# Lexmata/llama-gguf

Hardware: AMD Instinct MI355X
Metric: decode tokens/sec Llama-3-8B Q4_K_M, 1 GPU; % of HBM roofline (higher is better)
Workload: dtype f32 (x as 4xint8 limbs on the matrix cores, exact int32 accumulation)

## Files before the change

### include/llama_gguf_hip.h

```cpp
#ifndef LLAMA_GGUF_HIP_H
#define LLAMA_GGUF_HIP_H

#include <stddef.h>
#include <stdint.h>

#ifdef __cplusplus
extern "C" {
#endif

typedef enum lgh_status {
  LGH_OK = 0,
  LGH_NOT_AVAILABLE = 1,
  LGH_SHAPE_MISMATCH = 2,
  LGH_DTYPE_MISMATCH = 3,
  LGH_UNSUPPORTED_DTYPE = 4,
  LGH_UNSUPPORTED = 5,
  LGH_INVALID_ARGUMENT = 6,
  LGH_TENSOR_ERROR = 7,
  LGH_INITIALIZATION_FAILED = 8,
  LGH_ALLOCATION_FAILED = 9,
  LGH_OPERATION_FAILED = 10
} lgh_status;

typedef enum lgh_ggml_type {
// ... 29 lines not shown
enum {
  LGH_KV_F32 = 0,
  LGH_KV_INT8 = 1,
  LGH_KV_FP8_E4M3 = 2,
  LGH_KV_FP8_E5M2 = 3,
  LGH_KV_TQ2 = 4,
  LGH_KV_TQ3 = 5,
  LGH_KV_TQ2_QJL = 6,
  LGH_KV_TQ3_QJL = 7,
};

enum {
  LGH_FLAG_NO_GRAPH = 1u << 0,
  LGH_FLAG_EXACT_PREFILL = 1u << 2,
  LGH_FLAG_KV_INT8 = 1u << 4,
  LGH_FLAG_REMOVED_MASK = (1u << 1) | (1u << 3) | (1u << 5) | (1u << 6) | (1u << 7) | (0xFFu << 24),
  LGH_FLAG_ATTN_SPLITS_SHIFT = 8,
  LGH_FLAG_ATTN_DIRECT_SHIFT = 16
};

typedef struct lgh_ctx lgh_ctx;

enum {
  LGH_K_EMBED = 0, LGH_K_QKV = 1, LGH_K_ATTN = 2, LGH_K_ATTN_COMBINE = 3, LGH_K_WO = 4, LGH_K_GATEUP = 5,
  LGH_K_DOWN = 6, LGH_K_ROUTER = 7, LGH_K_OUTPUT = 8, LGH_K_ARGMAX = 9, LGH_K_MISC = 10,
  LGH_K_TOKEN = 11,
  LGH_K_COUNT = 16
};

enum {
  LGH_SYM_MV_Q4K = 0,
// ... 5 lines not shown
  LGH_SYM_MV_Q5K_Q6K = 6,
  LGH_SYM_MV_ALL = 7,
  LGH_SYM_F32_MATVEC = 8,
  LGH_SYM_ATTN = 9,
  LGH_SYM_ATTN_COMBINE = 10,
  LGH_SYM_EMBED = 11,
  LGH_SYM_ARGMAX = 12,
  LGH_SYM_ROUTER = 13,
  LGH_SYM_OTHER = 14,
  LGH_SYM_MVQ_Q4K = 15,
  LGH_SYM_MVQ_Q6K = 16,
  LGH_SYM_MVQ_MIXED = 17,
  LGH_SYM_MVQ_Q5K = 18,
  LGH_SYM_MVQ_Q80_Q40 = 19,
  LGH_SYM_PTOK = 20,
  LGH_SYM_COUNT = 24
};

typedef struct lgh_stats {
  uint64_t weight_bytes;
  uint64_t kv_bytes;
  uint64_t scratch_bytes;
  uint64_t tokens_processed;
  uint64_t graph_nodes;
  uint64_t k_launches[LGH_K_COUNT];
  double k_time_us[LGH_K_COUNT];
  uint64_t k_alg_bytes[LGH_K_COUNT];
  uint64_t sym_launches[LGH_SYM_COUNT];
  double sym_time_us[LGH_SYM_COUNT];
  uint64_t sym_alg_bytes[LGH_SYM_COUNT];
// ... 122 lines not shown
                            size_t n_kv_heads, size_t head_dim, size_t max_seq_len, float scale, size_t pos, int n_splits);
int lgh_op_attention_kv8(int device, uint32_t kv_cache_type, const float* q, int8_t* k_bytes, int8_t* v_bytes, float* k_scale, float* v_scale,
                         const float* k_new, const float* v_new, float* out, size_t n_heads, size_t n_kv_heads, size_t head_dim,
                         size_t max_seq_len, float scale, size_t pos, int n_splits);
int lgh_op_attention_tq(int device, uint32_t kv_cache_type, const float* q, uint8_t* k_codes, uint8_t* v_codes, uint32_t* k_qjl,
                        const float* k_new, const float* v_new, const float* signs, const float* qjl_matrices, float* out, size_t n_heads,
                        size_t n_kv_heads, size_t head_dim, size_t max_seq_len, float scale, size_t pos, int n_splits);
int lgh_op_attention_prefill(int device, const float* q, const float* k_cache, const float* v_cache, float* out, size_t n_heads,
                             size_t n_kv_heads, size_t head_dim, size_t max_seq_len, float scale, size_t pos0, size_t m_tokens);
int lgh_op_qkv_rope(int device, const uint32_t* types, const void* const* w, const float* const* bias, const float* x, const float* norm_w,
                    float eps, size_t hidden, size_t head_dim, size_t n_heads, size_t n_kv_heads, size_t max_seq_len, size_t pos,
                    float rope_base, float rope_scale, float* q_out, float* k_cache, float* v_cache);
int lgh_op_linear_chain(int device, uint32_t type_a, const void* w_a, const void* w_a_up, const float* bias_a, size_t k, size_t n_a,
                        const float* x, const float* norm_w, float eps, const float* resid, int xq_next, const float* next_nw,
                        uint32_t type_b, const void* w_b, size_t n_b, float* out_a, float* out_b, float* out_b_requant, int* image_used);
int lgh_op_moe_experts(int device, uint32_t type_gate_up, const void* w_gate, const void* w_up, uint32_t type_down, const void* w_down,
                       size_t n_experts, size_t hidden, size_t ffn, size_t top_k, const float* router, const int* sel, const float* sel_w,
                       const float* x, const float* norm_w, float eps, float* out, int* sel_out, float* sel_w_out);
typedef struct lgh_backend lgh_backend;
int lgh_backend_create(int device, lgh_backend** out);
void lgh_backend_destroy(lgh_backend* be);
int lgh_backend_load_weight(lgh_backend* be, const char* name, uint32_t ggml_type, const void* w, size_t k, size_t n);
int lgh_backend_has_weight(const lgh_backend* be, const char* name);
int lgh_backend_vec_mat_q(lgh_backend* be, const char* name, const float* x, float* out, size_t k, size_t n);
const char* lgh_backend_last_error(const lgh_backend* be);
int lgh_op_norm_vec_mat(int device, uint32_t ggml_type, const void* w, const float* x, const float* norm_w, float eps,
                        float* out, size_t k, size_t n);
int lgh_op_swiglu_vec_mat(int device, uint32_t ggml_type, const void* w_gate, const void* w_up, const float* x,
                          const float* norm_w, float eps, float* out, size_t k, size_t n);

// ... 31 lines not shown
```

### llama-gguf_amd/csrc/common.h

```cpp
#pragma once

#include <hip/hip_runtime.h>
#include <stdint.h>
#include <stddef.h>
#include <vector>

#include "../../include/llama_gguf_hip.h"

namespace lgh {

typedef uint32_t u32x4 __attribute__((ext_vector_type(4)));
typedef uint32_t u32x2 __attribute__((ext_vector_type(2)));
typedef float f32x4 __attribute__((ext_vector_type(4)));

constexpr int kWave = 64;
constexpr int kNumCU = 256;

__host__ __device__ inline uint32_t blk_elems(int t) {
  switch (t) {
    case LGH_TYPE_F32: case LGH_TYPE_F16: case LGH_TYPE_BF16: return 1;
    case LGH_TYPE_Q4_0: case LGH_TYPE_Q4_1: case LGH_TYPE_Q5_0: case LGH_TYPE_Q5_1: case LGH_TYPE_Q8_0:
    case LGH_TYPE_Q8_1: return 32;
    case LGH_TYPE_Q2_K: case LGH_TYPE_Q3_K: case LGH_TYPE_Q4_K: case LGH_TYPE_Q5_K: case LGH_TYPE_Q6_K:
    case LGH_TYPE_Q8_K: return 256;
// ... 98 lines not shown
  uint32_t ssq_stride;
  uint32_t out_stride[3];
  uint32_t resid_stride[3];
  uint32_t xq_out_stride[3];
  uint32_t ssq_out_stride[3];
  float* part;
  uint64_t part_floats;
  const int* ind_cnt;
  const int* ind_idx;
  uint32_t ind_div;
  uint32_t ind_stride;
  uint32_t ind_nz;
  uint64_t part_z_floats;
};

struct MvGeom { uint32_t wbpack, geom, geom2, red_floats, lds_red_off, n_wg; };

struct MvPlan {
  uint32_t units, T, G, rows_per_wg, n_wg, threads, red_floats;
};

hipError_t mv_plan(int dev_type, uint32_t k, uint32_t n_rows, int npass, MvPlan* plan, uint32_t launch_rows,
                   uint32_t wave_cap);
uint32_t mv_wave_cap(int dev_type);
hipError_t mv_launch(const MvLaunch& L, uint32_t n_wg, uint32_t threads, hipStream_t st);
int mv_symbol(const MvLaunch& L);
hipError_t mvq_plan(uint32_t k, uint32_t n_rows, int npass, MvPlan* plan, uint32_t launch_rows, uint32_t force_tiles = 0);
hipError_t mvq_launch(const MvLaunch& L, uint32_t n_wg, uint32_t threads, hipStream_t st);
hipError_t repack_q4k_t16_launch(const uint8_t* raw, uint8_t* dst, uint32_t n_rows, uint32_t nblk, hipStream_t st);
hipError_t hbm_read_launch(const uint8_t* buf, size_t bytes, float* sink, int nt, hipStream_t st);
uint32_t mvq_pack(const MvLaunch& L, uint32_t n_wg, uint32_t threads, MvGeom* g, size_t* lds_out);
uint32_t mvq_format_mask(const MvLaunch& L);
uint32_t mvq_tile_bytes(int dev_type);
hipError_t mvqb_launch(const MvLaunch& L, const MvBatch& B, uint32_t n_wg, uint32_t threads, hipStream_t st);
size_t mvqb_lds_bytes(uint32_t n_seq, uint32_t red_floats);
hipError_t xq_quantize_launch(const float* x, const float* nw, uint8_t* xq, float* ssq_part, uint32_t k, hipStream_t st);
hipError_t repack_t16_launch(int dev_type, const uint8_t* raw, uint8_t* dst, uint32_t n_rows, uint32_t nblk, hipStream_t st);
hipError_t repack_q6k_t16_launch(const uint8_t* raw, uint8_t* dst, uint32_t n_rows, uint32_t nblk, hipStream_t st);
hipError_t f32_matvec_launch(const float* w, const float* x, float* out, uint32_t k, uint32_t n, const float* norm_w,
                             float eps, const float* resid, hipStream_t st);

hipError_t repack_launch(int src_type, const uint8_t* raw, uint8_t* dst, const uint64_t plane_off[4], uint64_t n_blocks,
                         hipStream_t st);
// ... 74 lines not shown
```

### llama-gguf_amd/csrc/engine.h

```cpp
#pragma once

#include <string>
#include <vector>

#include "common.h"
#include "sample.h"

namespace lgh {

struct LayerW {
  bool owned = false;
  DevWeight wq, wk, wv, wo, gate, up, down;
  DevWeight gate_exps, up_exps, down_exps;
  float* attn_norm = nullptr;
  float* ffn_norm = nullptr;
  float* router = nullptr;
  float* bq = nullptr; float* bk = nullptr; float* bv = nullptr; float* bo = nullptr;
  float* kcache = nullptr;
  float* vcache = nullptr;
  int8_t *k8 = nullptr, *v8 = nullptr;
  float *kscale = nullptr, *vscale = nullptr;
  uint32_t* kx = nullptr;
  bool moe() const { return router != nullptr; }
};
// ... 59 lines not shown
  float* output_norm = nullptr;
  void *fwd_hidden = nullptr, *fwd_token = nullptr;
  float *hidden = nullptr, *xnorm = nullptr, *q = nullptr, *kv_tmp = nullptr, *attn_out = nullptr, *act = nullptr,
        *act2 = nullptr, *logits = nullptr, *part_ml = nullptr, *part_acc = nullptr, *rope_cs = nullptr, *moe_w = nullptr,
        *amax_v = nullptr;
  int *moe_sel = nullptr, *state = nullptr, *amax_i = nullptr, *tok_log = nullptr;
  uint32_t n_splits = 8;
  size_t pos = 0;
  bool finalized = false;
  bool profiling = false;
  std::string err;
  hipGraphExec_t graph[lgh::MODE_COUNT][2] = {};
  bool attn_direct = false;
  uint32_t direct_attn_max_kv = 0;
  uint64_t graph_nodes = 0;
  lgh_stats stats{};
  std::vector<lgh::ProfRec> prof;
  std::vector<void*> allocs;
  std::vector<lgh::XqBuf> xqs;
  lgh::PfScratch pf;
  lgh::BatchScratch batch;
  float* tq_signs = nullptr;
  std::vector<float> tq_signs_host;
  float* tq_qjl = nullptr;
  std::vector<float> tq_qjl_host;
  float* kv_shift_tmp = nullptr;
  lgh::SampBufs samp;
  lgh_sampler_config samp_cfg{};
  bool samp_set = false;
};
// ... 75 lines not shown
```

### llama-gguf_amd/csrc/engine.hip

```cpp
#include "engine.h"
#include "prefill.h"
#include "xq.h"

#include <algorithm>
#include <cmath>
#include <cstdio>
#include <cstdlib>
#include <cstring>

using namespace lgh;

namespace lgh {
hipError_t kv_store_launch(const float* k, const float* v, float* kcache, float* vcache, uint32_t n_kv, uint32_t d,
                           uint32_t max_seq, const int* pos, hipStream_t st);
}

int fail(lgh_ctx* c, int status, const std::string& msg) {
  if (c) c->err = msg;
  return status;
}

#define HIP_TRY(c, status, expr)                                                                      \
  do {                                                                                                \
    hipError_t e__ = (expr);                                                                          \
// ... 290 lines not shown
      } else if (qo && sp.epi != EPI_ROPE_K && sp.epi != EPI_V_CACHE) {
        qo->fresh = false;
      }
      if (sp.out2 && !S.xq_out2) xq_stale(c, sp.out2);
    }
    S.head_dim = c->d.head_dim;
    S.max_seq = c->d.max_seq_len;
    wg += plan.n_wg;
    if (plan.threads > threads) threads = plan.threads;
    if (plan.red_floats > L.red_floats) L.red_floats = plan.red_floats;
  }
  alg += (uint64_t)k * 4 * (norm_w ? 2 : 1);
  return LGH_OK;
}

static int mvq_symbol(const MvLaunch& L) {
  bool has[8] = {false, false, false, false, false, false, false, false};
  for (int s = 0; s < L.nseg; s++) {
    const int t = L.seg[s].type;
    has[t == kDevQ4K_T16 ? 0 : t == kDevQ6K_T16 ? 1 : t == kDevQ5K_T16 ? 2 : t == kDevQ80_T16 ? 3 : 4] = true;
  }
  return has[2] ? LGH_SYM_MVQ_Q5K : (has[3] || has[4]) ? LGH_SYM_MVQ_Q80_Q40 : (has[0] && has[1]) ? LGH_SYM_MVQ_MIXED
         : has[1] ? LGH_SYM_MVQ_Q6K : LGH_SYM_MVQ_Q4K;
}

static int launch_mv_group(lgh_ctx* c, int cls, const SegSpec* specs, int nseg, const float* norm_w, uint32_t k, bool mfma) {
  MvLaunch L;
  uint32_t wg, threads;
  uint64_t alg;
  int rc = build_mv_group(c, specs, nseg, norm_w, k, mfma, L, wg, threads, alg, 0);
  if (rc) return rc;
  if (mfma) return run_k(c, cls, mvq_symbol(L), alg, [&] { return mvq_launch(L, wg, threads, c->stream); });
  return run_k(c, cls, mv_symbol(L), alg, [&] { return mv_launch(L, wg, threads, c->stream); });
}

int launch_mv(lgh_ctx* c, int cls, const SegSpec* specs, int nseg, const float* norm_w, uint32_t k) {
  SegSpec a[3], b[3];
  int na = 0, nb = 0;
  for (int s = 0; s < nseg; s++) {
    if (mfma_type(specs[s].W[0]->type)) a[na++] = specs[s];
    else b[nb++] = specs[s];
  }
  int rc = LGH_OK;
  if (na > 1) {
    bool q4 = false, q5 = false, other = false;
    for (int s = 0; s < na; s++) {
      const int t = a[s].W[0]->type;
// ... 1251 lines not shown
```

### llama-gguf_amd/csrc/matvec_mfma.hip

```cpp
#include <algorithm>
#include <type_traits>

#include "device_utils.h"
#include "mv_epilogue.h"
#include "xq.h"
#include "mvq_core.h"
#include "timeline.h"

LGH_TL_DEFINE(mvq)

namespace lgh {

#ifdef LGH_STAMPS
__device__ unsigned long long g_stamps[8192 * 8];
hipError_t mvq_read_stamps(unsigned long long* host, size_t n) {
  return hipMemcpyFromSymbol(host, HIP_SYMBOL(g_stamps), n * sizeof(unsigned long long));
}
#define LGH_STAMP(i)                                                                             \
  do {                                                                                           \
    if (threadIdx.x == 0 && blockIdx.x < 8192) g_stamps[blockIdx.x * 8 + (i)] = __builtin_amdgcn_s_memrealtime(); \
  } while (0)
__device__ unsigned long long g_wstamps[2048 * 16 * 8];
hipError_t mvq_read_wave_stamps(unsigned long long* host, size_t n) {
  return hipMemcpyFromSymbol(host, HIP_SYMBOL(g_wstamps), n * sizeof(unsigned long long));
// ... 436 lines not shown
  mv_epilogue(L, S, wg, red, ssq, S_T, epi_pre);
  LGH_STAMP(5);
  LGH_WSTAMP(7);
  LGH_SPAN(1);
}

template <uint32_t MASK>
__global__ void __launch_bounds__(kWaves * 64) mvq_kernel(uint32_t wbpack, uint32_t geom, uint32_t geom2, uint32_t L_red_floats,
                                                          uint32_t lds_red_off, const MvLaunch L) {
  extern __shared__ __attribute__((aligned(16))) uint8_t smem8[];
  LGH_TL_BEGIN(mvq, lgh::TL_MVQ, geom2);
  mvq_body<MASK>(blockIdx.x, wbpack, geom, geom2, L_red_floats, lds_red_off, L, smem8);
  LGH_TL_END();
}

hipError_t mvq_plan(uint32_t k, uint32_t n_rows, int npass, MvPlan* plan, uint32_t launch_rows, uint32_t force_tiles) {
  if (k == 0 || k % 256 || n_rows == 0 || npass < 1 || npass > 4) return hipErrorInvalidValue;
  const uint32_t nblk = k / 256, W = kWaves;
  uint32_t T = 1;
  for (uint32_t t = 1; t <= W && t <= nblk; t++)
    if (nblk % t == 0) T = t;
  if (T < W / 2 && nblk > W) T = W;
  if (T > nblk) T = nblk;
  const uint32_t G = W / T >= 1 ? W / T : 1;
  const uint32_t nbw = (nblk + T - 1) / T;
  if (launch_rows < n_rows) launch_rows = n_rows;
  const uint32_t tiles_launch = (launch_rows + 15) / 16;
  uint32_t R = force_tiles ? force_tiles : (tiles_launch + kNumCU - 1) / kNumCU;
  R = (R + G - 1) / G * G;
  const uint32_t threads = T * G * 64;
  const uint32_t rmax = threads / 16 / G * G;
  if (R > rmax) R = rmax;
  plan->units = nbw;
  plan->T = T;
  plan->G = G;
  plan->rows_per_wg = 16 * R;
  plan->n_wg = ((n_rows + 15) / 16 + R - 1) / R;
  plan->threads = threads;
  plan->red_floats = (uint32_t)npass * T * 16 * R;
  return hipSuccess;
}

static uint32_t mvq_red_offset(uint32_t nwaves, uint32_t nbw) { return nwaves * nbw * kXqRecord; }
size_t mvq_lds_bytes(uint32_t nwaves, uint32_t nbw, uint32_t red_floats) {
  return (size_t)mvq_red_offset(nwaves, nbw) + (size_t)red_floats * 4 + 64;
}

template <uint32_t MASK>
static hipError_t mvq_go(const MvLaunch& L, uint32_t n_wg, uint32_t threads, size_t lds, hipStream_t st, uint32_t wbpack, uint32_t geom,
                         uint32_t geom2, uint32_t red_off) {
  static bool attr_set[64] = {};
  if (hipError_t e = lds_opt_in(reinterpret_cast<const void*>(&mvq_kernel<MASK>), 160 * 1024, attr_set); e != hipSuccess) return e;
  hipLaunchKernelGGL((mvq_kernel<MASK>), dim3(n_wg), dim3(threads), lds, st, wbpack, geom, geom2, L.red_floats, red_off, L);
  return hipGetLastError();
}

uint32_t mvq_pack(const MvLaunch& L, uint32_t n_wg, uint32_t threads, MvGeom* g, size_t* lds_out) {
  const MvSeg& S0 = L.seg[0];
  const size_t lds = mvq_lds_bytes(threads / 64, S0.units, L.red_floats);
  if (lds > 160 * 1024 || threads == 0 || threads > kWaves * 64 || n_wg == 0 || L.nseg < 1 || L.nseg > 3) return 0;
  uint32_t mask = 0;
  for (int i = 0; i < L.nseg; i++) {
    const MvSeg& Si = L.seg[i];
    if (Si.T != S0.T || Si.G != S0.G || Si.units != S0.units || Si.nblk != S0.nblk || Si.rows_per_wg % (16 * S0.G) ||
        (i > 0 && Si.wg_begin >= 0xFFFFu))
      return 0;
    const int f = fmt_of_dev_type(Si.type);
    if (f < 0) return 0;
    mask |= 1u << f;
  }
  const uint32_t Rg = S0.rows_per_wg / 16 / S0.G;
  if (S0.T > 255 || S0.G > 255 || S0.units > 0x3FFF || S0.nblk > 0xFFFF || Rg > 0xFFFF) return 0;
  g->wbpack = (L.nseg > 1 ? L.seg[1].wg_begin : 0xFFFFu) | (L.nseg > 2 ? L.seg[2].wg_begin : 0xFFFFu) << 16;
  g->geom = S0.T | S0.G << 8 | S0.units << 16 | (L.do_norm ? 1u << 31 : 0u);
  g->geom2 = S0.nblk | Rg << 16;
  g->red_floats = L.red_floats;
  g->lds_red_off = mvq_red_offset(threads / 64, S0.units);
  g->n_wg = n_wg;
  *lds_out = lds;
  return mask;
}

hipError_t mvq_launch(const MvLaunch& L, uint32_t n_wg, uint32_t threads, hipStream_t st) {
  MvGeom g;
  size_t lds = 0;
  const uint32_t mask = mvq_pack(L, n_wg, threads, &g, &lds);
  const uint32_t wbpack = g.wbpack, geom = g.geom, geom2 = g.geom2, red_off = g.lds_red_off;
#define LGH_MVQ_CASE(M) case M: return mvq_go<M>(L, n_wg, threads, lds, st, wbpack, geom, geom2, red_off)
  switch (mask) {
    LGH_MVQ_CASE(1u << F_Q4K); LGH_MVQ_CASE(1u << F_Q6K); LGH_MVQ_CASE(1u << F_Q5K); LGH_MVQ_CASE(1u << F_Q80); LGH_MVQ_CASE(1u << F_Q40);
    LGH_MVQ_CASE((1u << F_Q4K) | (1u << F_Q6K)); LGH_MVQ_CASE((1u << F_Q5K) | (1u << F_Q6K));
    default: return hipErrorInvalidValue;
  }
#undef LGH_MVQ_CASE
}

uint32_t mvq_tile_bytes(int dev_type) {
  const int f = fmt_of_dev_type(dev_type);
  return f < 0 ? 0u : fmt_tile_bytes(f);
}

uint32_t mvq_format_mask(const MvLaunch& L) {
// ... 11 lines not shown
```

### llama-gguf_amd/csrc/ops_api.hip

```cpp
#include "engine.h"
#include "prefill.h"

#include <cmath>
#include <vector>

using namespace lgh;

#include <algorithm>

#ifdef LGH_STAMPS
namespace lgh { hipError_t pf_read_stamps(unsigned long long* host, size_t n); }
extern "C" int lgh_debug_pf_stamps(unsigned long long* out, size_t n) { return lgh::pf_read_stamps(out, n) == hipSuccess ? 0 : 10; }
namespace lgh { hipError_t mv_read_stamps(unsigned long long* host, size_t n); hipError_t mvq_read_stamps(unsigned long long* host, size_t n); hipError_t mvq_read_wave_stamps(unsigned long long* host, size_t n); hipError_t mvq_spans(unsigned long long* host, int reset); }
#include <cstdio>
#include "timeline.h"
namespace lgh { hipError_t tl_read_mvq(void*); hipError_t tl_read_attn(void*); hipError_t tl_read_deq(void*); hipError_t tl_read_misc(void*); }
extern "C" long long lgh_debug_timeline(int which, void* out) {
  if (!out) return (long long)sizeof(lgh::TlBuf);
  hipError_t e = which == 0 ? lgh::tl_read_mvq(out) : which == 1 ? lgh::tl_read_attn(out) : which == 2 ? lgh::tl_read_deq(out) : lgh::tl_read_misc(out);
  return e == hipSuccess ? 0 : -1;
}
#endif

namespace {

struct Tmp {
  lgh_ctx* c = nullptr;
  int rc = LGH_OK;
  explicit Tmp(int device) {
    int n = lgh_device_count();
    if (n <= 0 || device < 0 || device >= n) { rc = LGH_NOT_AVAILABLE; return; }
    c = new lgh_ctx();
    c->device = device;
    c->d.norm_eps = 1e-5f;
    if (hipSetDevice(device) != hipSuccess || hipStreamCreateWithFlags(&c->own_stream, hipStreamNonBlocking) != hipSuccess) {
      rc = LGH_INITIALIZATION_FAILED;
      delete c;
      c = nullptr;
      return;
    }
    c->stream = c->own_stream;
    if ((rc = dev_alloc(c, (void**)&c->state, ST_WORDS * 4))) return;
    (void)hipMemsetAsync(c->state, 0, ST_WORDS * 4, c->stream);
  }
  ~Tmp() {
    if (!c) return;
    (void)hipStreamSynchronize(c->stream);
    for (void* p : c->allocs) (void)hipFree(p);
    (void)hipStreamDestroy(c->own_stream);
    delete c;
  }
  float* up(const float* host, size_t n) {
    float* d = nullptr;
    if (dev_alloc(c, (void**)&d, n * 4)) return nullptr;
    if (host && hipMemcpyAsync(d, host, n * 4, hipMemcpyHostToDevice, c->stream) != hipSuccess) return nullptr;
    return d;
  }
  int down(float* host, const float* dev, size_t n) {
    if (hipMemcpyAsync(host, dev, n * 4, hipMemcpyDeviceToHost, c->stream) != hipSuccess) return LGH_OPERATION_FAILED;
    return hipStreamSynchronize(c->stream) == hipSuccess ? LGH_OK : LGH_OPERATION_FAILED;
  }
};
// ... 790 lines not shown
    sp.xq_next = xq_next; sp.xq_next_nw = dnext;
    if ((rc = launch_mv(t.c, LGH_K_GATEUP, &sp, 1, dnw, (uint32_t)k))) return rc;
  } else if ((rc = linear_any(t.c, LGH_K_MISC, WA, dx, da, dnw, dres, dbias, xq_next, dnext))) {
    return rc;
  }
  qa = xq_get(t.c, da, (uint32_t)n_a);
  if (image_used) *image_used = qa && qa->fresh ? 1 : 0;
  const float* bnw = xq_next == 2 ? dnext : nullptr;
  if ((rc = linear_any(t.c, LGH_K_MISC, WB, da, db, bnw, nullptr, nullptr))) return rc;
  xq_stale(t.c, da);
  if ((rc = linear_any(t.c, LGH_K_MISC, WB, da, db2, bnw, nullptr, nullptr))) return rc;
  if ((rc = t.down(out_a, da, n_a)) || (rc = t.down(out_b, db, n_b))) return rc;
  return t.down(out_b_requant, db2, n_b);
}

int lgh_op_moe_experts(int device, uint32_t type_gate_up, const void* w_gate, const void* w_up, uint32_t type_down, const void* w_down,
                       size_t n_experts, size_t hidden, size_t ffn, size_t top_k, const float* router, const int* sel, const float* sel_w,
                       const float* x, const float* norm_w, float eps, float* out, int* sel_out, float* sel_w_out) {
  Tmp t(device);
  if (t.rc) return t.rc;
  if (!w_gate || !w_up || !w_down || !x || !norm_w || !out || (!router && (!sel || !sel_w)) || top_k == 0 || top_k > 8 ||
      top_k > n_experts || n_experts > 64)
    return LGH_INVALID_ARGUMENT;
  if (sel)
    for (size_t i = 0; i < top_k; i++)
      if (sel[i] < 0 || (size_t)sel[i] >= n_experts) return LGH_INVALID_ARGUMENT;
  lgh_model_desc& d = t.c->d;
  d.norm_eps = eps;
  d.hidden_size = (uint32_t)hidden;
  d.num_experts = (uint32_t)n_experts;
// ... 25 lines not shown
```

### llama-gguf_amd/hip_backend.py

```python
from __future__ import annotations

import ctypes as C
import os
from typing import Iterable, Optional, Sequence

import numpy as np

_HERE = os.path.dirname(os.path.abspath(__file__))
LIB_PATH = os.path.join(_HERE, "lib", "libllama_gguf_hip%s.so" % ("_" + os.environ["LGH_LIB_VARIANT"] if os.environ.get("LGH_LIB_VARIANT") else ""))

ABI_SYMBOLS = (
    "lgh_device_count", "lgh_create", "lgh_upload_tensor", "lgh_finalize", "lgh_destroy", "lgh_forward",
    "lgh_prefill_token", "lgh_prefill_batch", "lgh_prefill_is_batched", "lgh_op_mat_mat",
    "lgh_op_kv_roundtrip", "lgh_op_add", "lgh_op_mul", "lgh_op_scale", "lgh_op_silu", "lgh_op_gelu", "lgh_op_softmax", "lgh_op_matmul", "lgh_op_matvec",
    "lgh_op_matvec_q", "lgh_op_attention", "lgh_backend_create", "lgh_backend_destroy", "lgh_backend_load_weight",
    "lgh_backend_has_weight", "lgh_backend_vec_mat_q", "lgh_backend_last_error", "lgh_reset", "lgh_position", "lgh_kv_truncate", "lgh_kv_shift_left", "lgh_stage_prefill_batch", "lgh_stage_hidden_block_buffer", "lgh_forward_argmax", "lgh_decode_greedy",
    "lgh_last_error", "lgh_get_stats", "lgh_set_profiling", "lgh_set_stream", "lgh_get_stream", "lgh_synchronize",
    "lgh_read_hidden", "lgh_stage_hidden_buffer", "lgh_stage_forward", "lgh_op_dequantize", "lgh_op_vec_mat",
    "lgh_op_rms_norm", "lgh_op_rope", "lgh_op_attention_cached", "lgh_op_silu_mul", "lgh_op_norm_vec_mat",
    "lgh_op_swiglu_vec_mat", "lgh_bench_vec_mat", "lgh_bench_hbm_read", "lgh_gguf_inspect", "lgh_load_gguf",
    "lgh_stage_io_buffers", "lgh_stage_set_forward_targets", "lgh_stage_step", "lgh_stage_read_tokens", "lgh_gguf_get", "lgh_stage_read_logits",
    "lgh_pipeline_create", "lgh_pipeline_upload_tensor", "lgh_pipeline_finalize", "lgh_pipeline_destroy", "lgh_pipeline_forward",
    "lgh_pipeline_prefill_token", "lgh_pipeline_decode_greedy", "lgh_pipeline_reset", "lgh_pipeline_position", "lgh_pipeline_kv_truncate", "lgh_pipeline_stages",
    "lgh_pipeline_last_error",
    "lgh_set_kv_rotation_signs", "lgh_op_tq_compress", "lgh_set_kv_qjl_matrices", "lgh_op_tq_compress_qjl",
    "lgh_batch_create", "lgh_batch_reset", "lgh_batch_position", "lgh_batch_prefill", "lgh_forward_multi", "lgh_decode_greedy_multi",
    "lgh_set_sampler", "lgh_decode_sample", "lgh_batch_set_sampler", "lgh_decode_sample_multi", "lgh_op_sample",
    "lgh_op_attention_decode", "lgh_op_attention_kv8", "lgh_op_attention_tq", "lgh_op_attention_prefill",
    "lgh_op_qkv_rope", "lgh_op_linear_chain", "lgh_op_moe_experts",
)

K_NAMES = ("embed", "qkv", "attn", "attn_combine", "wo", "gate_up", "down", "router", "output", "argmax", "misc", "token")
K_COUNT = 16
SYM_COUNT = 24
SYM_NAMES = ("lgh::mv_kernel<1u, 1024>", "lgh::mv_kernel<8u, 1024>", "lgh::mv_kernel<16u, 1024>",
             "lgh::mv_kernel<2u, 768>", "lgh::mv_kernel<4u, 512>", "lgh::mv_kernel<5u, 512>", "lgh::mv_kernel<6u, 512>",
             "lgh::mv_kernel<31u, 512>", "lgh::f32_matvec_kernel", "lgh::attn_partial_kernel", "lgh::attn_combine_kernel",
             "lgh::embed_kernel", "lgh::argmax_stage1+2", "lgh::moe_router_kernel", "other", "lgh::mvq_kernel<1u>", "lgh::mvq_kernel<2u>", "lgh::mvq_kernel<3u>", "lgh::mvq_kernel<4u>",
             "lgh::mvq_kernel<8u>", "unused")
FLAG_NO_GRAPH = 1
FLAG_EXACT_PREFILL = 4
KV_F32, KV_INT8, KV_FP8_E4M3, KV_FP8_E5M2 = 0, 1, 2, 3
KV_TQ2, KV_TQ3 = 4, 5
KV_TQ2_QJL, KV_TQ3_QJL = 6, 7
FLAG_KV_INT8 = 16
FLAG_REMOVED_MASK = 2 | 8 | 32 | 64 | 128 | (0xFF << 24)


class BackendError(RuntimeError):
    VARIANTS = {1: "NotAvailable", 2: "ShapeMismatch", 3: "DTypeMismatch", 4: "UnsupportedDType", 5: "Unsupported",
                6: "InvalidArgument", 7: "Tensor", 8: "InitializationFailed", 9: "AllocationFailed",
                10: "OperationFailed"}

    def __init__(self, status: int, message: str = ""):
        self.status = status
        self.variant = self.VARIANTS.get(status, f"Status{status}")
        super().__init__(f"{self.variant}: {message}" if message else self.variant)


class ModelDesc(C.Structure):
    _fields_ = ([(n, C.c_uint32) for n in (
# ... 110 lines not shown
        "lgh_batch_create": (C.c_int, [vp, u32]), "lgh_batch_reset": (C.c_int, [vp, u32]), "lgh_batch_position": (sz, [vp, u32]),
        "lgh_batch_prefill": (C.c_int, [vp, u32, vp, sz]), "lgh_forward_multi": (C.c_int, [vp, vp, vp, u32, vp, vp]),
        "lgh_decode_greedy_multi": (C.c_int, [vp, vp, vp, u32, sz, vp]),
        "lgh_set_sampler": (C.c_int, [vp, C.POINTER(SamplerConfig)]),
        "lgh_decode_sample": (C.c_int, [vp, u32, vp, sz, sz, vp, vp]),
        "lgh_batch_set_sampler": (C.c_int, [vp, u32, C.POINTER(SamplerConfig)]),
        "lgh_decode_sample_multi": (C.c_int, [vp, vp, vp, u32, vp, vp, sz, vp, vp]),
        "lgh_op_sample": (C.c_int, [C.c_int, vp, sz, C.POINTER(SamplerConfig), vp, sz, vp, f32, C.POINTER(u32)]),
        "lgh_op_attention_decode": (C.c_int, [C.c_int, C.c_int, vp, vp, vp, vp, sz, sz, sz, sz, f32, sz, C.c_int]),
        "lgh_op_attention_kv8": (C.c_int, [C.c_int, u32, vp, vp, vp, vp, vp, vp, vp, vp, sz, sz, sz, sz, f32, sz, C.c_int]),
        "lgh_op_attention_tq": (C.c_int, [C.c_int, u32, vp, vp, vp, vp, vp, vp, vp, vp, vp, sz, sz, sz, sz, f32, sz, C.c_int]),
        "lgh_op_attention_prefill": (C.c_int, [C.c_int, vp, vp, vp, vp, sz, sz, sz, sz, f32, sz, sz]),
        "lgh_op_qkv_rope": (C.c_int, [C.c_int, vp, vp, vp, vp, vp, f32, sz, sz, sz, sz, sz, sz, f32, f32, vp, vp, vp]),
        "lgh_op_linear_chain": (C.c_int, [C.c_int, u32, vp, vp, vp, sz, sz, vp, vp, f32, vp, C.c_int, vp, u32, vp, sz, vp, vp, vp,
                                          C.POINTER(C.c_int)]),
        "lgh_op_moe_experts": (C.c_int, [C.c_int, u32, vp, vp, u32, vp, sz, sz, sz, sz, vp, vp, vp, vp, vp, f32, vp, vp, vp]),
    }
    for name, (res, args) in sig.items():
        fn = getattr(L, name)
        fn.restype, fn.argtypes = res, args
    _lib = L
    return L


def device_count() -> int:
    return load_library().lgh_device_count()


def _f32(a) -> np.ndarray:
    return np.ascontiguousarray(a, dtype=np.float32)
# ... 453 lines not shown

def op_linear_chain(type_a: int, w_a, k: int, n_a: int, x, type_b: int, w_b, n_b: int, *, w_a_up=None, bias_a=None, norm_w=None,
                    eps: float = 1e-5, resid=None, xq_next: int = 0, next_nw=None, device: int = 0):
    x = _f32(x)
    wa, wb = np.ascontiguousarray(w_a, dtype=np.uint8), np.ascontiguousarray(w_b, dtype=np.uint8)
    wu = None if w_a_up is None else np.ascontiguousarray(w_a_up, dtype=np.uint8)
    ba, nw, rs, nn = (None if v is None else _f32(v) for v in (bias_a, norm_w, resid, next_nw))
    oa, ob, ob2 = np.empty(n_a, np.float32), np.empty(n_b, np.float32), np.empty(n_b, np.float32)
    used = C.c_int(-1)
    _chk(load_library().lgh_op_linear_chain(device, type_a, wa.ctypes.data, _ptr(wu), _ptr(ba), k, n_a, x.ctypes.data, _ptr(nw), eps,
                                            _ptr(rs), xq_next, _ptr(nn), type_b, wb.ctypes.data, n_b, oa.ctypes.data, ob.ctypes.data,
                                            ob2.ctypes.data, C.byref(used)), "linear_chain")
    return oa, ob, ob2, bool(used.value)


def op_moe_experts(type_gate_up: int, w_gate, w_up, type_down: int, w_down, n_experts: int, hidden: int, ffn: int, top_k: int, x,
                   norm_w, eps: float, *, router=None, sel=None, sel_w=None, device: int = 0):
    x, nw = _f32(x), _f32(norm_w)
    wg, wu, wd = (np.ascontiguousarray(w, dtype=np.uint8) for w in (w_gate, w_up, w_down))
    r = None if router is None else _f32(router)
    s = None if sel is None else np.ascontiguousarray(sel, dtype=np.int32)
    sw = None if sel_w is None else _f32(sel_w)
    out, so, swo = np.empty(hidden, np.float32), np.empty(top_k, np.int32), np.empty(top_k, np.float32)
    _chk(load_library().lgh_op_moe_experts(device, type_gate_up, wg.ctypes.data, wu.ctypes.data, type_down, wd.ctypes.data, n_experts,
                                           hidden, ffn, top_k, _ptr(r), _ptr(s), _ptr(sw), x.ctypes.data, nw.ctypes.data, eps,
                                           out.ctypes.data, so.ctypes.data, swo.ctypes.data), "moe_experts")
    return out, so, swo


def op_attention_kv8(kv_cache_type: int, q, k_bytes, v_bytes, k_scale, v_scale, k_new, v_new, scale: float, pos: int, n_splits: int = 8,
# ... 277 lines not shown
```

Before: 611.2.

## Add 4-wave MFMA matvec kernel where each wave handles two k-slices

Adds a 256-thread variant of the quantized MFMA matvec, used by default for eligible launches (T=8, G=1, single pass, few tiles per workgroup). Each wave owns two k-slice roles, issues all tile loads for both up front and waits on vmcnt before consuming them. The aim is to cut per-workgroup wave count and scheduling overhead while keeping enough memory requests in flight. It also adds debug and opt-out flags, a test op that exports the xq image, and a wave-count query. The cost is more registers per wave, and each wave carries double the load on its own.

```diff
diff --git a/include/llama_gguf_hip.h b/include/llama_gguf_hip.h
--- a/include/llama_gguf_hip.h
+++ b/include/llama_gguf_hip.h
@@ -67,7 +67,10 @@
   LGH_FLAG_NO_GRAPH = 1u << 0,
   LGH_FLAG_EXACT_PREFILL = 1u << 2,
   LGH_FLAG_KV_INT8 = 1u << 4,
-  LGH_FLAG_REMOVED_MASK = (1u << 1) | (1u << 3) | (1u << 5) | (1u << 6) | (1u << 7) | (0xFFu << 24),
+  LGH_FLAG_REMOVED_MASK = (1u << 1) | (1u << 3) | (1u << 5) | (1u << 6) | (1u << 7) | (0x0Fu << 24),
+  LGH_FLAG_DBG_MV_W8_SINGLE = 1u << 28,
+  LGH_FLAG_DBG_MV_W8_FUSED = 1u << 29,
+  LGH_FLAG_MV_W8_ONLY = 1u << 30,
   LGH_FLAG_ATTN_SPLITS_SHIFT = 8,
   LGH_FLAG_ATTN_DIRECT_SHIFT = 16
 };
@@ -103,6 +106,7 @@
   LGH_SYM_MVQ_Q5K = 18,
   LGH_SYM_MVQ_Q80_Q40 = 19,
   LGH_SYM_PTOK = 20,
+  LGH_SYM_MVQ_W4 = 21,
   LGH_SYM_COUNT = 24
 };
 
@@ -255,6 +259,11 @@
 int lgh_op_linear_chain(int device, uint32_t type_a, const void* w_a, const void* w_a_up, const float* bias_a, size_t k, size_t n_a,
                         const float* x, const float* norm_w, float eps, const float* resid, int xq_next, const float* next_nw,
                         uint32_t type_b, const void* w_b, size_t n_b, float* out_a, float* out_b, float* out_b_requant, int* image_used);
+int lgh_op_linear_image(int device, uint32_t type, const void* w, const float* bias, size_t k, size_t n, const float* x,
+                        const float* norm_w, float eps, const float* resid, int xq_next, const float* next_nw, float* out,
+                        uint8_t* xq_image, size_t* image_bytes, float* ssq_out);
+void lgh_op_set_flags(uint32_t flags);
+uint32_t lgh_op_last_mv_waves(void);
 int lgh_op_moe_experts(int device, uint32_t type_gate_up, const void* w_gate, const void* w_up, uint32_t type_down, const void* w_down,
                        size_t n_experts, size_t hidden, size_t ffn, size_t top_k, const float* router, const int* sel, const float* sel_w,
                        const float* x, const float* norm_w, float eps, float* out, int* sel_out, float* sel_w_out);
diff --git a/llama-gguf_amd/csrc/common.h b/llama-gguf_amd/csrc/common.h
--- a/llama-gguf_amd/csrc/common.h
+++ b/llama-gguf_amd/csrc/common.h
@@ -136,7 +136,7 @@
   uint64_t part_z_floats;
 };
 
-struct MvGeom { uint32_t wbpack, geom, geom2, red_floats, lds_red_off, n_wg; };
+struct MvGeom { uint32_t wbpack, geom, geom2, red_floats, lds_red_off, n_wg, waves; };
 
 struct MvPlan {
   uint32_t units, T, G, rows_per_wg, n_wg, threads, red_floats;
@@ -149,6 +149,7 @@
 int mv_symbol(const MvLaunch& L);
 hipError_t mvq_plan(uint32_t k, uint32_t n_rows, int npass, MvPlan* plan, uint32_t launch_rows, uint32_t force_tiles = 0);
 hipError_t mvq_launch(const MvLaunch& L, uint32_t n_wg, uint32_t threads, hipStream_t st);
+bool mvq_w4_eligible(const MvLaunch& L);
 hipError_t repack_q4k_t16_launch(const uint8_t* raw, uint8_t* dst, uint32_t n_rows, uint32_t nblk, hipStream_t st);
 hipError_t hbm_read_launch(const uint8_t* buf, size_t bytes, float* sink, int nt, hipStream_t st);
 uint32_t mvq_pack(const MvLaunch& L, uint32_t n_wg, uint32_t threads, MvGeom* g, size_t* lds_out);
diff --git a/llama-gguf_amd/csrc/engine.h b/llama-gguf_amd/csrc/engine.h
--- a/llama-gguf_amd/csrc/engine.h
+++ b/llama-gguf_amd/csrc/engine.h
@@ -97,6 +97,7 @@
   bool attn_direct = false;
   uint32_t direct_attn_max_kv = 0;
   uint64_t graph_nodes = 0;
+  uint32_t last_mv_waves = 0;
   lgh_stats stats{};
   std::vector<lgh::ProfRec> prof;
   std::vector<void*> allocs;
diff --git a/llama-gguf_amd/csrc/engine.hip b/llama-gguf_amd/csrc/engine.hip
--- a/llama-gguf_amd/csrc/engine.hip
+++ b/llama-gguf_amd/csrc/engine.hip
@@ -328,7 +328,8 @@
   return LGH_OK;
 }
 
-static int mvq_symbol(const MvLaunch& L) {
+static int mvq_symbol(const MvLaunch& L, uint32_t threads) {
+  if (threads == 256 && L.seg[0].T * L.seg[0].G == 8) return LGH_SYM_MVQ_W4;
   bool has[8] = {false, false, false, false, false, false, false, false};
   for (int s = 0; s < L.nseg; s++) {
     const int t = L.seg[s].type;
@@ -344,7 +345,13 @@
   uint64_t alg;
   int rc = build_mv_group(c, specs, nseg, norm_w, k, mfma, L, wg, threads, alg, 0);
   if (rc) return rc;
-  if (mfma) return run_k(c, cls, mvq_symbol(L), alg, [&] { return mvq_launch(L, wg, threads, c->stream); });
+  if (mfma) {
+    bool w4 = !(c->d.flags & LGH_FLAG_MV_W8_ONLY) && mvq_w4_eligible(L);
+    if (w4 && (c->d.flags & (nseg > 1 ? LGH_FLAG_DBG_MV_W8_FUSED : LGH_FLAG_DBG_MV_W8_SINGLE))) w4 = false;
+    if (w4) threads = 256;
+    c->last_mv_waves = threads / 64;
+    return run_k(c, cls, mvq_symbol(L, threads), alg, [&] { return mvq_launch(L, wg, threads, c->stream); });
+  }
   return run_k(c, cls, mv_symbol(L), alg, [&] { return mv_launch(L, wg, threads, c->stream); });
 }
 
diff --git a/llama-gguf_amd/csrc/matvec_mfma.hip b/llama-gguf_amd/csrc/matvec_mfma.hip
--- a/llama-gguf_amd/csrc/matvec_mfma.hip
+++ b/llama-gguf_amd/csrc/matvec_mfma.hip
@@ -474,6 +474,174 @@
   LGH_TL_END();
 }
 
+constexpr int kWaves4 = 4;
+constexpr int kItems4 = 4;
+
+template <int N>
+__device__ __forceinline__ void mvq_wait_behind() {
+  static_assert(N >= 0 && N < 64, "vmcnt is a 6-bit counter");
+  asm volatile("s_waitcnt vmcnt(%0)" ::"n"(N) : "memory");
+}
+
+template <uint32_t MASK>
+__device__ __forceinline__ void mvq_body_w4(const uint32_t bid, uint32_t wbpack, uint32_t geom, uint32_t geom2, uint32_t L_red_floats,
+                                            uint32_t lds_red_off, const MvLaunch& L, uint8_t* smem8) {
+  const int* L_pos = L.pos;
+  uint32_t pos_now;
+  asm volatile("s_load_dword %0, %1, 0x0" : "=s"(pos_now) : "s"(L_pos) : "memory");
+  const int s = (int)(bid >= (wbpack & 0xFFFFu)) + (int)(bid >= (wbpack >> 16));
+  const MvSeg& S = L.seg[s];
+  const uint32_t S_nrows = S.n_rows, S_wgb = S.wg_begin, S_head_dim = S.head_dim;
+  const int S_epi = S.epi;
+  const float* S_resid = S.resid;
+  const float* S_xq_nw = S.xq_nw;
+  const float* L_rope_cs = L.rope_cs;
+  constexpr bool kSingle = (MASK & (MASK - 1)) == 0;
+  const int fmt = kSingle ? __builtin_ctz(MASK) : fmt_of_dev_type(S.type);
+  auto is = [&](int f) { return ((MASK >> f) & 1u) != 0 && (kSingle || fmt == f); };
+  const uint32_t tb = is(F_Q4K) ? fmt_tile_bytes(F_Q4K) : is(F_Q6K) ? fmt_tile_bytes(F_Q6K) : is(F_Q5K) ? fmt_tile_bytes(F_Q5K)
+                      : is(F_Q80) ? fmt_tile_bytes(F_Q80) : fmt_tile_bytes(F_Q40);
+  const uint32_t S_T = geom & 0xFFu, nbw = (geom >> 16) & 0x3FFFu;
+  const bool nrm = (geom >> 31) != 0;
+  const uint32_t S_nblk = geom2 & 0xFFFFu;
+  const uint32_t Rg = L.nseg > 1 ? S.rows_per_wg >> 4 : geom2 >> 16;
+  const uint32_t S_rpw = 16u * Rg;
+  const uint32_t wg = bid - S_wgb;
+
+  const uint32_t tid = threadIdx.x, lane = tid & 63;
+  const uint32_t wave = __builtin_amdgcn_readfirstlane(tid >> 6);
+  LGH_SPAN(0);
+  const uint32_t ksA = wave, ksB = wave + kWaves4;
+  const uint32_t blk0A = ksA * nbw, blk0B = ksB * nbw;
+  uint32_t nblkA = blk0A < S_nblk ? min(nbw, S_nblk - blk0A) : 0;
+  uint32_t nblkB = blk0B < S_nblk ? min(nbw, S_nblk - blk0B) : 0;
+  const uint32_t ntiles = (S_nrows + 15) >> 4;
+  const uint32_t tile0 = wg * Rg;
+  uint32_t ntile_w = tile0 < ntiles ? min(Rg, ntiles - tile0) : 0;
+  const uint32_t lds_base = (uint32_t)(uintptr_t)(__attribute__((address_space(3))) uint8_t*)smem8;
+  const uint8_t* xrecA = smem8 + blk0A * kXqRecord;
+  const uint8_t* xrecB = smem8 + blk0B * kXqRecord;
+  float* red = reinterpret_cast<float*>(smem8 + lds_red_off);
+  float* ssq = red + L_red_floats;
+  const uint32_t n = lane & 15, mq = lane >> 4;
+
+  const MvPass& P = S.pass[0];
+  const uint8_t* pbase = P.plane[0] + (uint64_t)tile0 * S_nblk * tb;
+  const uint8_t* px = P.xq;
+  const float* L_ssq_part = L.ssq_part;
+  const uint32_t L_n_ssq = L.n_ssq_part;
+  float ssp[4] = {0.0f, 0.0f, 0.0f, 0.0f};
+  if (nrm && wave == 0) {
+#pragma unroll
+    for (int j = 0; j < 4; j++)
+      if (lane + 64 * j < L_n_ssq) ssp[j] = L_ssq_part[lane + 64 * j];
+  }
+  MvEpiPre epi_pre = {0.0f, 0.0f, false};
+  mv_epilogue_prefetch_resid(S_epi, S_resid, S_xq_nw, S_nrows, wg, S_rpw, epi_pre);
+  asm volatile("s_waitcnt lgkmcnt(0)" : "+s"(pos_now));
+  mv_epilogue_prefetch_rope(S_epi, pos_now, L_rope_cs, S_head_dim, S_nrows, wg, S_rpw, epi_pre);
+  LGH_STAMP(0);
+  asm volatile("" : "+s"(nblkA), "+s"(nblkB), "+s"(ntile_w));
+  const uint32_t nA = ntile_w * nblkA, nB = ntile_w * nblkB;
+
+  auto x_request = [&](uint32_t blk0, uint32_t nblk_r) {
+    for (uint32_t b = 0; b < nblk_r; b++) {
+      const uint8_t* src = px + (size_t)(blk0 + b) * kXqRecord;
+      const uint32_t dst = lds_base + (blk0 + b) * kXqRecord;
+      uint32_t keep;
+      asm volatile("s_mov_b32 %0, m0\n\ts_mov_b32 m0, %3\n\ts_nop 0\n\tglobal_load_lds_dwordx4 %1, off\n\ts_add_u32 m0, m0, 0x400\n\t"
+                   "s_nop 0\n\tglobal_load_lds_dword %2, off\n\ts_mov_b32 m0, %0"
+                   : "=&s"(keep) : "v"(src + lane * 16), "v"(src + 1024 + lane * 4), "s"(dst) : "memory");
+    }
+  };
+  struct Pos { uint32_t tl, b; };
+  auto issue = [&](uint32_t blk0, const Pos& q, RawT16& r) {
+    mvq_issue_tile<MASK>(fmt, pbase + ((size_t)q.tl * S_nblk + blk0 + q.b) * tb, lane, r);
+  };
+  auto consume = [&](const uint8_t* xrec, uint32_t ks, uint32_t nblk_r, const Pos& q, const RawT16& r, float& acc) {
+    mvq_consume_tile<MASK>(fmt, r, xrec + q.b * kXqRecord, lane, acc);
+    if (q.b + 1 == nblk_r) {
+      float t = acc + __shfl_xor(acc, 16, 64);
+      t += __shfl_xor(t, 32, 64);
+      if (mq == 0) red[(size_t)ks * S_rpw + q.tl * 16 + n] = t;
+      acc = 0.0f;
+    }
+  };
+  auto zero_slots = [&](uint32_t ks) {
+    for (uint32_t tl = 0; tl < ntile_w; tl++)
+      if (mq == 0) red[(size_t)ks * S_rpw + tl * 16 + n] = 0.0f;
+  };
+
+  x_request(blk0A, nblkA);
+  x_request(blk0B, nblkB);
+  RawT16 bufA[kItems4], bufB[kItems4];
+  Pos posA[kItems4], posB[kItems4];
+  Pos nxA = {0, 0}, nxB = {0, 0};
+  float accA = 0.0f, accB = 0.0f;
+  auto run = [&](auto n_each) {
+    constexpr int N = decltype(n_each)::value;
+#pragma unroll
+    for (int j = 0; j < N; j++) {
+      posA[j] = nxA; issue(blk0A, nxA, bufA[j]); if (++nxA.b == nblkA) { nxA.b = 0; ++nxA.tl; }
+      posB[j] = nxB; issue(blk0B, nxB, bufB[j]); if (++nxB.b == nblkB) { nxB.b = 0; ++nxB.tl; }
+    }
+    if (is(F_Q6K) || is(F_Q80)) mvq_wait_behind<2 * N * 5>();
+    else if (is(F_Q5K)) mvq_wait_behind<2 * N * 4>();
+    else mvq_wait_behind<2 * N * 3>();
+#pragma unroll
+    for (int j = 0; j < N; j++) {
+      consume(xrecA, ksA, nblkA, posA[j], bufA[j], accA);
+      consume(xrecB, ksB, nblkB, posB[j], bufB[j], accB);
+    }
+  };
+  if (nA == nB && nA == 1) {
+    run(std::integral_constant<int, 1>{});
+  } else if (nA == nB && nA == 2) {
+    run(std::integral_constant<int, 2>{});
+  } else if (nA == nB && nA == 3) {
+    run(std::integral_constant<int, 3>{});
+  } else if (nA == nB && nA == 4) {
+    run(std::integral_constant<int, 4>{});
+  } else {
+#pragma unroll
+    for (int j = 0; j < kItems4; j++) {
+      if ((uint32_t)j < nA) { posA[j] = nxA; issue(blk0A, nxA, bufA[j]); if (++nxA.b == nblkA) { nxA.b = 0; ++nxA.tl; } }
+      if ((uint32_t)j < nB) { posB[j] = nxB; issue(blk0B, nxB, bufB[j]); if (++nxB.b == nblkB) { nxB.b = 0; ++nxB.tl; } }
+    }
+    mvq_wait_behind<0>();
+#pragma unroll
+    for (int j = 0; j < kItems4; j++) {
+      if ((uint32_t)j < nA) consume(xrecA, ksA, nblkA, posA[j], bufA[j], accA);
+      if ((uint32_t)j < nB) consume(xrecB, ksB, nblkB, posB[j], bufB[j], accB);
+    }
+    if (nblkA == 0) zero_slots(ksA);
+    if (nblkB == 0) zero_slots(ksB);
+  }
+  LGH_STAMP(3);
+  if (nrm && wave == 0) {
+    float ss = (ssp[0] + ssp[1]) + (ssp[2] + ssp[3]);
+    for (uint32_t i = 256 + lane; i < L_n_ssq; i += 64) ss += L_ssq_part[i];
+    ss = wave_sum_to_lane63(ss);
+    if (lane == 63) ssq[0] = ss;
+  } else if (nrm && lane == 0) {
+    ssq[wave] = 0.0f;
+  }
+  __syncthreads();
+  LGH_STAMP(4);
+  mv_epilogue(L, S, wg, red, ssq, S_T, epi_pre);
+  LGH_STAMP(5);
+  LGH_SPAN(1);
+}
+
+template <uint32_t MASK>
+__global__ void __launch_bounds__(kWaves4 * 64) mvq_w4_kernel(uint32_t wbpack, uint32_t geom, uint32_t geom2, uint32_t L_red_floats,
+                                                              uint32_t lds_red_off, const MvLaunch L) {
+  extern __shared__ __attribute__((aligned(16))) uint8_t smem8[];
+  LGH_TL_BEGIN(mvq, lgh::TL_MVQ, geom2);
+  mvq_body_w4<MASK>(blockIdx.x, wbpack, geom, geom2, L_red_floats, lds_red_off, L, smem8);
+  LGH_TL_END();
+}
+
 hipError_t mvq_plan(uint32_t k, uint32_t n_rows, int npass, MvPlan* plan, uint32_t launch_rows, uint32_t force_tiles) {
   if (k == 0 || k % 256 || n_rows == 0 || npass < 1 || npass > 4) return hipErrorInvalidValue;
   const uint32_t nblk = k / 256, W = kWaves;
@@ -501,9 +669,22 @@
   return hipSuccess;
 }
 
-static uint32_t mvq_red_offset(uint32_t nwaves, uint32_t nbw) { return nwaves * nbw * kXqRecord; }
-size_t mvq_lds_bytes(uint32_t nwaves, uint32_t nbw, uint32_t red_floats) {
-  return (size_t)mvq_red_offset(nwaves, nbw) + (size_t)red_floats * 4 + 64;
+static uint32_t mvq_red_offset(uint32_t nroles, uint32_t nbw) { return nroles * nbw * kXqRecord; }
+size_t mvq_lds_bytes(uint32_t nroles, uint32_t nbw, uint32_t red_floats) {
+  return (size_t)mvq_red_offset(nroles, nbw) + (size_t)red_floats * 4 + 64;
+}
+
+bool mvq_w4_eligible(const MvLaunch& L) {
+  if (L.nseg < 1 || L.nseg > 3) return false;
+  for (int i = 0; i < L.nseg; i++) {
+    const MvSeg& S = L.seg[i];
+    if (S.T != 8 || S.G != 1 || S.npass != 1 || S.pass[0].sel) return false;
+    if (S.rows_per_wg % 16 || (S.rows_per_wg / 16) * S.units > (uint32_t)kItems4) return false;
+    if (S.epi != EPI_STORE && S.epi != EPI_RESID && S.epi != EPI_ROPE_Q && S.epi != EPI_ROPE_K && S.epi != EPI_V_CACHE) return false;
+  }
+  const uint32_t m = mvq_format_mask(L);
+  const bool single = m != 0 && (m & (m - 1)) == 0;
+  return single || m == ((1u << F_Q4K) | (1u << F_Q6K)) || m == ((1u << F_Q5K) | (1u << F_Q6K));
 }
 
 template <uint32_t MASK>
@@ -515,13 +696,26 @@
   return hipGetLastError();
 }
 
+template <uint32_t MASK>
+static hipError_t mvq_go_w4(const MvLaunch& L, uint32_t n_wg, size_t lds, hipStream_t st, uint32_t wbpack, uint32_t geom, uint32_t geom2,
+                            uint32_t red_off) {
+  static bool attr_set[64] = {};
+  if (hipError_t e = lds_opt_in(reinterpret_cast<const void*>(&mvq_w4_kernel<MASK>), 160 * 1024, attr_set); e != hipSuccess) return e;
+  hipLaunchKernelGGL((mvq_w4_kernel<MASK>), dim3(n_wg), dim3(kWaves4 * 64), lds, st, wbpack, geom, geom2, L.red_floats, red_off, L);
+  return hipGetLastError();
+}
+
 uint32_t mvq_pack(const MvLaunch& L, uint32_t n_wg, uint32_t threads, MvGeom* g, size_t* lds_out) {
   const MvSeg& S0 = L.seg[0];
-  const size_t lds = mvq_lds_bytes(threads / 64, S0.units, L.red_floats);
+  const uint32_t roles = S0.T * S0.G;
+  const size_t lds = mvq_lds_bytes(roles, S0.units, L.red_floats);
   if (lds > 160 * 1024 || threads == 0 || threads > kWaves * 64 || n_wg == 0 || L.nseg < 1 || L.nseg > 3) return 0;
+  if (threads != roles * 64 && !(threads == kWaves4 * 64 && mvq_w4_eligible(L))) return 0;
   uint32_t mask = 0;
   for (int i = 0; i < L.nseg; i++) {
     const MvSeg& Si = L.seg[i];
+    const bool pairs = Si.epi == EPI_ROPE_Q || Si.epi == EPI_ROPE_K;
+    if ((pairs ? (Si.rows_per_wg + 1) / 2 : Si.rows_per_wg) > threads) return 0;
     if (Si.T != S0.T || Si.G != S0.G || Si.units != S0.units || Si.nblk != S0.nblk || Si.rows_per_wg % (16 * S0.G) ||
         (i > 0 && Si.wg_begin >= 0xFFFFu))
       return 0;
@@ -535,8 +729,9 @@
   g->geom = S0.T | S0.G << 8 | S0.units << 16 | (L.do_norm ? 1u << 31 : 0u);
   g->geom2 = S0.nblk | Rg << 16;
   g->red_floats = L.red_floats;
-  g->lds_red_off = mvq_red_offset(threads / 64, S0.units);
+  g->lds_red_off = mvq_red_offset(roles, S0.units);
   g->n_wg = n_wg;
+  g->waves = threads / 64;
   *lds_out = lds;
   return mask;
 }
@@ -546,6 +741,15 @@
   size_t lds = 0;
   const uint32_t mask = mvq_pack(L, n_wg, threads, &g, &lds);
   const uint32_t wbpack = g.wbpack, geom = g.geom, geom2 = g.geom2, red_off = g.lds_red_off;
+  if (mask && g.waves == (uint32_t)kWaves4 && (geom & 0xFFu) * ((geom >> 8) & 0xFFu) == (uint32_t)kWaves) {
+#define LGH_MVQ_CASE(M) case M: return mvq_go_w4<M>(L, n_wg, lds, st, wbpack, geom, geom2, red_off)
+    switch (mask) {
+      LGH_MVQ_CASE(1u << F_Q4K); LGH_MVQ_CASE(1u << F_Q6K); LGH_MVQ_CASE(1u << F_Q5K); LGH_MVQ_CASE(1u << F_Q80); LGH_MVQ_CASE(1u << F_Q40);
+      LGH_MVQ_CASE((1u << F_Q4K) | (1u << F_Q6K)); LGH_MVQ_CASE((1u << F_Q5K) | (1u << F_Q6K));
+      default: return hipErrorInvalidValue;
+    }
+#undef LGH_MVQ_CASE
+  }
 #define LGH_MVQ_CASE(M) case M: return mvq_go<M>(L, n_wg, threads, lds, st, wbpack, geom, geom2, red_off)
   switch (mask) {
     LGH_MVQ_CASE(1u << F_Q4K); LGH_MVQ_CASE(1u << F_Q6K); LGH_MVQ_CASE(1u << F_Q5K); LGH_MVQ_CASE(1u << F_Q80); LGH_MVQ_CASE(1u << F_Q40);
diff --git a/llama-gguf_amd/csrc/ops_api.hip b/llama-gguf_amd/csrc/ops_api.hip
--- a/llama-gguf_amd/csrc/ops_api.hip
+++ b/llama-gguf_amd/csrc/ops_api.hip
@@ -1,5 +1,6 @@
 #include "engine.h"
 #include "prefill.h"
+#include "xq.h"
 
 #include <cmath>
 #include <vector>
@@ -24,6 +25,9 @@
 
 namespace {
 
+uint32_t g_op_flags = 0;
+uint32_t g_last_mv_waves = 0;
+
 struct Tmp {
   lgh_ctx* c = nullptr;
   int rc = LGH_OK;
@@ -33,6 +37,7 @@
     c = new lgh_ctx();
     c->device = device;
     c->d.norm_eps = 1e-5f;
+    c->d.flags = g_op_flags;
     if (hipSetDevice(device) != hipSuccess || hipStreamCreateWithFlags(&c->own_stream, hipStreamNonBlocking) != hipSuccess) {
       rc = LGH_INITIALIZATION_FAILED;
       delete c;
@@ -46,6 +51,7 @@
   ~Tmp() {
     if (!c) return;
     (void)hipStreamSynchronize(c->stream);
+    if (c->last_mv_waves) g_last_mv_waves = c->last_mv_waves;
     for (void* p : c->allocs) (void)hipFree(p);
     (void)hipStreamDestroy(c->own_stream);
     delete c;
@@ -866,6 +872,41 @@
   return t.down(out_b_requant, db2, n_b);
 }
 
+void lgh_op_set_flags(uint32_t flags) { g_op_flags = flags; }
+uint32_t lgh_op_last_mv_waves(void) { return g_last_mv_waves; }
+
+int lgh_op_linear_image(int device, uint32_t type, const void* w, const float* bias, size_t k, size_t n, const float* x,
+                        const float* norm_w, float eps, const float* resid, int xq_next, const float* next_nw, float* out,
+                        uint8_t* xq_image, size_t* image_bytes, float* ssq_out) {
+  Tmp t(device);
+  if (t.rc) return t.rc;
+  if (!w || !x || !out || xq_next < 0 || xq_next > 2 || (xq_next == 2 && !next_nw)) return LGH_INVALID_ARGUMENT;
+  t.c->d.norm_eps = eps;
+  const size_t nb = weight_bytes(type, k, n);
+  if (!nb) return LGH_SHAPE_MISMATCH;
+  DevWeight W;
+  int rc;
+  if ((rc = upload_matrix(t.c, W, (int)type, (uint32_t)k, (uint32_t)n, 1, -1, w, nb))) return rc;
+  float *dx = t.up(x, k), *dnw = norm_w ? t.up(norm_w, k) : nullptr, *dres = resid ? t.up(resid, n) : nullptr;
+  float *dbias = bias ? t.up(bias, n) : nullptr, *dnext = next_nw ? t.up(next_nw, n) : nullptr, *dout = t.up(nullptr, n);
+  if (!dx || (norm_w && !dnw) || (resid && !dres) || (bias && !dbias) || (next_nw && !dnext) || !dout) return LGH_ALLOCATION_FAILED;
+  const uint32_t nq = (uint32_t)((n + 255) / 256 * 256);
+  XqBuf* q0 = xq_get(t.c, dout, nq);
+  if (!q0) return LGH_ALLOCATION_FAILED;
+  if (hipMemsetAsync(q0->xq, 0, xq_bytes(nq), t.c->stream) != hipSuccess) return LGH_OPERATION_FAILED;
+  if ((rc = linear_any(t.c, LGH_K_MISC, W, dx, dout, dnw, dres, dbias, xq_next, dnext))) return rc;
+  XqBuf* q = xq_get(t.c, dout, nq);
+  const bool left = q && q->fresh && xq_next;
+  if (image_bytes) *image_bytes = 0;
+  if (left && xq_image) {
+    const size_t bytes = xq_bytes(nq);
+    if (hipMemcpyAsync(xq_image, q->xq, bytes, hipMemcpyDeviceToHost, t.c->stream) != hipSuccess) return LGH_OPERATION_FAILED;
+    if (image_bytes) *image_bytes = bytes;
+  }
+  if (left && xq_next == 2 && ssq_out && (rc = t.down(ssq_out, q->ssq, n / 16))) return rc;
+  return t.down(out, dout, n);
+}
+
 int lgh_op_moe_experts(int device, uint32_t type_gate_up, const void* w_gate, const void* w_up, uint32_t type_down, const void* w_down,
                        size_t n_experts, size_t hidden, size_t ffn, size_t top_k, const float* router, const int* sel, const float* sel_w,
                        const float* x, const float* norm_w, float eps, float* out, int* sel_out, float* sel_w_out) {
diff --git a/llama-gguf_amd/hip_backend.py b/llama-gguf_amd/hip_backend.py
--- a/llama-gguf_amd/hip_backend.py
+++ b/llama-gguf_amd/hip_backend.py
@@ -28,6 +28,7 @@
     "lgh_set_sampler", "lgh_decode_sample", "lgh_batch_set_sampler", "lgh_decode_sample_multi", "lgh_op_sample",
     "lgh_op_attention_decode", "lgh_op_attention_kv8", "lgh_op_attention_tq", "lgh_op_attention_prefill",
     "lgh_op_qkv_rope", "lgh_op_linear_chain", "lgh_op_moe_experts",
+    "lgh_op_linear_image", "lgh_op_set_flags", "lgh_op_last_mv_waves",
 )
 
 K_NAMES = ("embed", "qkv", "attn", "attn_combine", "wo", "gate_up", "down", "router", "output", "argmax", "misc", "token")
@@ -37,14 +38,16 @@
              "lgh::mv_kernel<2u, 768>", "lgh::mv_kernel<4u, 512>", "lgh::mv_kernel<5u, 512>", "lgh::mv_kernel<6u, 512>",
              "lgh::mv_kernel<31u, 512>", "lgh::f32_matvec_kernel", "lgh::attn_partial_kernel", "lgh::attn_combine_kernel",
              "lgh::embed_kernel", "lgh::argmax_stage1+2", "lgh::moe_router_kernel", "other", "lgh::mvq_kernel<1u>", "lgh::mvq_kernel<2u>", "lgh::mvq_kernel<3u>", "lgh::mvq_kernel<4u>",
-             "lgh::mvq_kernel<8u>", "unused")
+             "lgh::mvq_kernel<8u>", "unused", "lgh::mvq_w4_kernel")
 FLAG_NO_GRAPH = 1
 FLAG_EXACT_PREFILL = 4
 KV_F32, KV_INT8, KV_FP8_E4M3, KV_FP8_E5M2 = 0, 1, 2, 3
 KV_TQ2, KV_TQ3 = 4, 5
 KV_TQ2_QJL, KV_TQ3_QJL = 6, 7
 FLAG_KV_INT8 = 16
-FLAG_REMOVED_MASK = 2 | 8 | 32 | 64 | 128 | (0xFF << 24)
+FLAG_MV_W8_ONLY = 1 << 30
+FLAG_DBG_MV_W8_SINGLE, FLAG_DBG_MV_W8_FUSED = 1 << 28, 1 << 29
+FLAG_REMOVED_MASK = 2 | 8 | 32 | 64 | 128 | (0x0F << 24)
 
 
 class BackendError(RuntimeError):
@@ -185,6 +188,8 @@
         "lgh_op_qkv_rope": (C.c_int, [C.c_int, vp, vp, vp, vp, vp, f32, sz, sz, sz, sz, sz, sz, f32, f32, vp, vp, vp]),
         "lgh_op_linear_chain": (C.c_int, [C.c_int, u32, vp, vp, vp, sz, sz, vp, vp, f32, vp, C.c_int, vp, u32, vp, sz, vp, vp, vp,
                                           C.POINTER(C.c_int)]),
+        "lgh_op_linear_image": (C.c_int, [C.c_int, u32, vp, vp, sz, sz, vp, vp, f32, vp, C.c_int, vp, vp, vp, C.POINTER(sz), vp]),
+        "lgh_op_set_flags": (None, [u32]), "lgh_op_last_mv_waves": (u32, []),
         "lgh_op_moe_experts": (C.c_int, [C.c_int, u32, vp, vp, u32, vp, sz, sz, sz, sz, vp, vp, vp, vp, vp, f32, vp, vp, vp]),
     }
     for name, (res, args) in sig.items():
@@ -668,6 +673,29 @@
     return oa, ob, ob2, bool(used.value)
 
 
+def op_linear_image(ggml_type: int, w, k: int, n: int, x, *, bias=None, norm_w=None, eps: float = 1e-5, resid=None, xq_next: int = 0,
+                    next_nw=None, device: int = 0):
+    x, wa = _f32(x), np.ascontiguousarray(w, dtype=np.uint8)
+    ba, nw, rs, nn = (None if v is None else _f32(v) for v in (bias, norm_w, resid, next_nw))
+    out = np.empty(n, np.float32)
+    img = np.zeros((n + 255) // 256 * 1280, np.uint8)
+    ssq = np.zeros(n // 16, np.float32)
+    nbytes = C.c_size_t(0)
+    _chk(load_library().lgh_op_linear_image(device, ggml_type, wa.ctypes.data, _ptr(ba), k, n, x.ctypes.data, _ptr(nw), eps, _ptr(rs),
+                                            xq_next, _ptr(nn), out.ctypes.data, img.ctypes.data, C.byref(nbytes), ssq.ctypes.data),
+         "linear_image")
+    left = nbytes.value > 0
+    return out, (img[:nbytes.value] if left else None), (ssq if left and xq_next == 2 else None)
+
+
+def op_set_flags(flags: int) -> None:
+    load_library().lgh_op_set_flags(flags)
+
+
+def op_last_mv_waves() -> int:
+    return int(load_library().lgh_op_last_mv_waves())
+
+
 def op_moe_experts(type_gate_up: int, w_gate, w_up, type_down: int, w_down, n_experts: int, hidden: int, ffn: int, top_k: int, x,
                    norm_w, eps: float, *, router=None, sel=None, sel_w=None, device: int = 0):
     x, nw = _f32(x), _f32(norm_w)
```

Measured after the change: 595.4. 2.6% lower.
